# Amanda-Zheng/MR-GNAS

Hardware: AMD Instinct MI355X
Metric: million edges/sec per supernet fwd+bwd step (FB15k-237, dim=200) (higher is better)
Workload: dtype f32

## Files before the change

### mr-gnas_amd/csrc/mixedop.hip

```cpp
#include "common.hpp"

#define MRG_MIX_MAXK 8
static_assert(MRG_MIX_MAXK == MRG_MIX_MAX_CANDIDATES, "mrg_gated_branch.given is sized by the header's constant");

namespace mrg {

struct PtrPack { const float* p[MRG_MIX_MAXK]; };
struct MutPack { float* p[MRG_MIX_MAXK]; };
struct RowScalePack { const float* rs[MRG_MIX_MAXK]; float scale[MRG_MIX_MAXK]; float self_scale[MRG_MIX_MAXK]; int64_t edge_rows[MRG_MIX_MAXK]; int on[MRG_MIX_MAXK];
                      const float* full[MRG_MIX_MAXK];
                      const float* s[MRG_MIX_MAXK]; const float* gate[MRG_MIX_MAXK]; float* gs_out[MRG_MIX_MAXK]; int add_from[MRG_MIX_MAXK]; };

struct GatedPack { int k; const float* s; const float* c;
                   int pair_k;
                   int rk; const float* rf;
                   const float* rh; const float* uvc; int uld; int64_t b0, b1; float* rdq;
                   const int32_t* vrows;
                   int act; };

__device__ __forceinline__ int64_t valid_rows(const int32_t* vrows, int64_t rows) {
  if (vrows == nullptr) return rows;
  const int64_t v = (int64_t)*vrows;
  return v < rows ? (v < 0 ? 0 : v) : rows;
}
// ... 262 lines not shown
#pragma unroll
        for (int k = 0; k < KB; ++k) {
          vin[k] = Vec<VEC>::fill(0.f);
          if (k < K && ys.p[k]) vin[k] = Vec<VEC>::load(ys.p[k] + r * D + c * VEC);
        }
#pragma unroll
        for (int k = 0; k < KB; ++k) {
          if (k < K) {
            Vec<VEC> v = vin[k];
            if constexpr (GATED) {
              const bool isg = k == gp.k;
              const float cm = isg ? gck : (k == gp.rk ? rfv : 1.0f);
#pragma unroll
              for (int j = 0; j < VEC; ++j) v[j] = v[j] * (isg ? gsv[j] : 1.0f) * cm;
            }
            Vec<VEC> sc = Vec<VEC>::load(lds + (k * 2 + 0) * D + c * VEC), sh = Vec<VEC>::load(lds + (k * 2 + 1) * D + c * VEC);
            if constexpr (ACT == 0) {
#pragma unroll
              for (int j = 0; j < VEC; ++j) {
                float z = v[j] * sc[j] + sh[j];
                acc[j] += wk[k] * (z > 0.f ? z : 0.f);
              }
            } else {
#pragma unroll
              for (int j = 0; j < VEC; ++j) acc[j] += wk[k] * tanhf(v[j] * sc[j] + sh[j]);
            }
          }
        }
        if (pad) acc = Vec<VEC>::fill(0.f);
        acc.store(out + r * D + c * VEC);
      }
    }
  }
}

template <int VEC, int LPR, int KMAX, int KB, bool GATED, int ACT = 0>
__global__ __launch_bounds__(MRG_BLOCK) void mix_bwd_reduce_k(const float* __restrict__ g, PtrPack ys, int K,
                                                              const float* __restrict__ coef, const float* __restrict__ w,
                                                              float* __restrict__ ws, int64_t rows, int D, GatedPack gp) {
  rows = valid_rows(gp.vrows, rows);
  extern __shared__ float lds[];
  constexpr int RPB = MRG_BLOCK / LPR;
  constexpr int WIDTH = LPR * KMAX * VEC;
  const int sl = threadIdx.x % LPR, rw = row_group_of_thread<LPR>();
  const int dv = D / VEC;
  float* red = lds + K * 4 * D;
  for (int t = threadIdx.x; t < K * 4 * D; t += MRG_BLOCK) lds[t] = coef[t];
  __syncthreads();
  float wk[KB];
  Vec<VEC> a0[KB][KMAX], a1[KB][KMAX], a2[KB][KMAX];
#pragma unroll
  for (int k = 0; k < KB; ++k) {
    wk[k] = k < K ? w[k] : 0.f;
#pragma unroll
    for (int q = 0; q < KMAX; ++q) { a0[k][q] = Vec<VEC>::fill(0.f); a1[k][q] = Vec<VEC>::fill(0.f); a2[k][q] = Vec<VEC>::fill(0.f); }
  }
  for (int64_t r = (int64_t)blockIdx.x * RPB + rw; r < rows; r += (int64_t)gridDim.x * RPB) {
#pragma unroll
    for (int q = 0; q < KMAX; ++q) {
      int c = sl + q * LPR;
      if (c < dv) {
        float gck = 1.f, rfv = 1.f;
        Vec<VEC> gsv = Vec<VEC>::fill(0.f);
        if constexpr (GATED) {
          gck = gated_rowscale(gp, r);
          rfv = gp.rf[r];
          gsv = Vec<VEC>::load(gp.s + r * D + c * VEC);
        }
        Vec<VEC> gv = Vec<VEC>::load(g + r * D + c * VEC);
        Vec<VEC> vin[KB];
#pragma unroll
        for (int k = 0; k < KB; ++k) {
          vin[k] = Vec<VEC>::fill(0.f);
          if (k < K && ys.p[k]) vin[k] = Vec<VEC>::load(ys.p[k] + r * D + c * VEC);
        }
#pragma unroll
        for (int k = 0; k < KB; ++k) {
          if (k < K) {
            Vec<VEC> v = vin[k];
            if constexpr (GATED) {
              const bool isg = k == gp.k;
              const float cm = isg ? gck : (k == gp.rk ? rfv : 1.0f);
#pragma unroll
              for (int j = 0; j < VEC; ++j) v[j] = v[j] * (isg ? gsv[j] : 1.0f) * cm;
            }
            const float* cf = lds + k * 4 * D + c * VEC;
            const Vec<VEC> c0 = Vec<VEC>::load(cf), c1 = Vec<VEC>::load(cf + D), c2 = Vec<VEC>::load(cf + 2 * D), c3 = Vec<VEC>::load(cf + 3 * D);
#pragma unroll
            for (int j = 0; j < VEC; ++j) {
              float z = v[j] * c0[j] + c1[j];
              float xh = v[j] * c2[j] - c3[j];
              float rl, gr;
              if constexpr (ACT == 0) { rl = z > 0.f ? z : 0.f; gr = z > 0.f ? wk[k] * gv[j] : 0.f; }
              else { rl = tanhf(z); gr = wk[k] * gv[j] * (1.f - rl * rl); }
              a0[k][q][j] += gr;
              a1[k][q][j] += gr * xh;
              a2[k][q][j] += gv[j] * rl;
            }
          }
        }
      }
    }
  }
#pragma unroll
  for (int k = 0; k < KB; ++k) {
    if (k < K) {
      __syncthreads();
#pragma unroll
      for (int q = 0; q < KMAX; ++q) {
        int c = sl + q * LPR;
#pragma unroll
        for (int j = 0; j < VEC; ++j) {
          red[(rw * 3 + 0) * WIDTH + c * VEC + j] = a0[k][q][j];
          red[(rw * 3 + 1) * WIDTH + c * VEC + j] = a1[k][q][j];
          red[(rw * 3 + 2) * WIDTH + c * VEC + j] = a2[k][q][j];
        }
      }
      __syncthreads();
      float* dst = ws + ((int64_t)blockIdx.x * K + k) * 3 * D;
      for (int t = threadIdx.x; t < 3 * D; t += MRG_BLOCK) {
        int which = t / D, c = t - which * D;
        float acc = 0.f;
#pragma unroll
        for (int q2 = 0; q2 < RPB; ++q2) acc += red[(q2 * 3 + which) * WIDTH + c];
        dst[t] = acc;
      }
    }
  }
}

__global__ void mix_finalize_bwd_k(const float* __restrict__ red, int K, double total_rows, int D, float* __restrict__ coef2,
                                   MutPack dgamma, MutPack dbeta, float* __restrict__ dw, const int32_t* __restrict__ vrows) {
  if (vrows) total_rows = *vrows > 0 ? (double)*vrows : 1.0;
  __shared__ float part[256];
  int k = blockIdx.x;
  float accw = 0.f;
  for (int c = threadIdx.x; c < D; c += blockDim.x) {
    float s0 = red[(k * 3 + 0) * D + c], s1 = red[(k * 3 + 1) * D + c];
    coef2[(k * 2 + 0) * D + c] = (float)(s0 / total_rows);
    coef2[(k * 2 + 1) * D + c] = (float)(s1 / total_rows);
    if (dgamma.p[k]) dgamma.p[k][c] = s1;
    if (dbeta.p[k]) dbeta.p[k][c] = s0;
    accw += red[(k * 3 + 2) * D + c];
  }
  part[threadIdx.x] = accw;
  __syncthreads();
  if (threadIdx.x == 0) {
    float tot = 0.f;
    for (int i = 0; i < (int)blockDim.x; ++i) tot += part[i];
    dw[k] = tot;
  }
}

template <int VEC, int LPR, int KMAX, bool GATED, int KB, int ACT = 0>
__global__ __launch_bounds__(MRG_BLOCK) void mix_bwd_apply_k(const float* __restrict__ g, PtrPack ys, MutPack gys, int K,
                                                             const float* __restrict__ coef, const float* __restrict__ coef2,
                                                             const float* __restrict__ w, int64_t rows, int D, RowScalePack rsp,
                                                             GatedPack gp) {
  extern __shared__ float lds[];
  constexpr int RPB = MRG_BLOCK / LPR;
  const int sl = threadIdx.x % LPR, rw = row_group_of_thread<LPR>();
  const int dv = D / VEC;
  for (int t = threadIdx.x; t < K * 6 * D; t += MRG_BLOCK) {
    int k = t / (6 * D), rem = t - k * 6 * D;
    lds[t] = rem < 4 * D ? coef[(int64_t)k * 4 * D + rem] : coef2[(int64_t)k * 2 * D + rem - 4 * D];
  }
  __syncthreads();
  float wk[KB];
  bool need[KB];
#pragma unroll
  for (int k = 0; k < KB; ++k) {
    wk[k] = k < K ? w[k] : 0.f;
    need[k] = k < K && (gys.p[k] != nullptr || (GATED && k == gp.rk));
  }
#pragma unroll
  for (int k = 0; k < KB; ++k)
    if (k < K && rsp.on[k] == 2 && rsp.add_from[k] >= 0) {
#pragma unroll
      for (int q = 0; q < KB; ++q) if (q == rsp.add_from[k]) need[q] = true;
    }
  const bool hasr = GATED && gp.rk >= 0;
  const int64_t nvalid = valid_rows(gp.vrows, rows);
  for (int64_t r = (int64_t)blockIdx.x * RPB + rw; r < rows; r += (int64_t)gridDim.x * RPB) {
    const float live = r < nvalid ? 1.0f : 0.0f;
#pragma unroll
    for (int q = 0; q < KMAX; ++q) {
      const int c = sl + q * LPR;
      const bool act = c < dv;
      float gck = 1.f, rfv = 1.f, rhv = 0.f;
      Vec<VEC> gsv = Vec<VEC>::fill(0.f), gga = Vec<VEC>::fill(0.f), guv = Vec<VEC>::fill(0.f);
      Vec<VEC> ov[KB];
      Vec<VEC> orv = Vec<VEC>::fill(0.f);
      float dq = 0.f;
      float ckv[KB];
#pragma unroll
      for (int k = 0; k < KB; ++k) ckv[k] = 1.f;
      if (act) {
        if constexpr (GATED) {
          gck = gated_rowscale(gp, r);
          rfv = gp.rf[r];
          rhv = gp.rh[r];
          gsv = Vec<VEC>::load(gp.s + r * D + c * VEC);
          const int seg = (r >= gp.b0) + (r >= gp.b1);
          guv = Vec<VEC>::load(gp.uvc + (int64_t)seg * gp.uld + c * VEC);
        }
        Vec<VEC> gv = Vec<VEC>::load(g + r * D + c * VEC);
        Vec<VEC> vin[KB];
#pragma unroll
        for (int k = 0; k < KB; ++k) {
          vin[k] = Vec<VEC>::fill(0.f);
          if (k < K && need[k] && ys.p[k]) vin[k] = Vec<VEC>::load(ys.p[k] + r * D + c * VEC);
          if (k < K && rsp.on[k] && rsp.full[k]) ckv[k] = rsp.full[k][r];
        }
        if constexpr (GATED) {
#pragma unroll
          for (int k = 0; k < KB; ++k) {
            if (k == gp.k) {
              gga = vin[k];
#pragma unroll
              for (int j = 0; j < VEC; ++j) vin[k][j] = vin[k][j] * gsv[j] * gck;
            }
            if (k == gp.rk) {
#pragma unroll
              for (int j = 0; j < VEC; ++j) vin[k][j] = vin[k][j] * rfv;
            }
          }
        }
#pragma unroll
        for (int k = 0; k < KB; ++k) {
          ov[k] = Vec<VEC>::fill(0.f);
          if (k < K && need[k]) {
            const Vec<VEC> v = vin[k];
            const float* cf = lds + k * 6 * D + c * VEC;
            const Vec<VEC> c0 = Vec<VEC>::load(cf), c1 = Vec<VEC>::load(cf + D), c2 = Vec<VEC>::load(cf + 2 * D),
                           c3 = Vec<VEC>::load(cf + 3 * D), c4 = Vec<VEC>::load(cf + 4 * D), c5 = Vec<VEC>::load(cf + 5 * D);
#pragma unroll
            for (int j = 0; j < VEC; ++j) {
              float z = v[j] * c0[j] + c1[j];
              float xh = v[j] * c2[j] - c3[j];
              float gr;
              if constexpr (ACT == 0) gr = z > 0.f ? wk[k] * gv[j] : 0.f;
              else { const float th = tanhf(z); gr = wk[k] * gv[j] * (1.f - th * th); }
              ov[k][j] = (gr - c4[j] - xh * c5[j]) * c0[j] * live;
            }
          }
        }
        if (hasr) {
#pragma unroll
          for (int k = 0; k < KB; ++k) if (k == gp.rk) orv = ov[k];
#pragma unroll
          for (int j = 0; j < VEC; ++j) dq += orv[j] * gsv[j];
        }
      }
      float dzr = 0.f;
      if (hasr) {
        const float qr = group_sum<LPR>(dq);
        dzr = qr * rhv;
        if (sl == 0) gp.rdq[r] = qr;
      }
      if (act) {
#pragma unroll
        for (int k = 0; k < KB; ++k) {
          if (k < K && gys.p[k] != nullptr) {
            Vec<VEC> o = ov[k];
            if (rsp.on[k]) {
              const float ck = rsp.full[k] ? ckv[k]
                                           : (r < rsp.edge_rows[k] ? rsp.scale[k] * (rsp.rs[k] ? rsp.rs[k][r] : 1.0f) : rsp.self_scale[k]);
              if (rsp.on[k] == 2) {
                const Vec<VEC> sv = (GATED && k == gp.k) ? gsv : Vec<VEC>::load(rsp.s[k] + r * D + c * VEC);
                const Vec<VEC> ga = (GATED && k == gp.k) ? gga : Vec<VEC>::load(rsp.gate[k] + r * D + c * VEC);
                Vec<VEC> o2;
#pragma unroll
                for (int j = 0; j < VEC; ++j) {
                  const float gc = o[j] * ck;
                  o2[j] = gc * ga[j];
                  o[j] = gc * sv[j] * ga[j] * (1.0f - ga[j]);
                }
                const int af = rsp.add_from[k];
                if (af >= 0) {
#pragma unroll
                  for (int qq = 0; qq < KB; ++qq)
                    if (qq == af) {
#pragma unroll
                      for (int j = 0; j < VEC; ++j) o2[j] += ov[qq][j];
                    }
                }
                if (hasr && k == gp.k) {
#pragma unroll
                  for (int j = 0; j < VEC; ++j) o2[j] += orv[j] * rfv + dzr * guv[j];
                }
                o2.store(rsp.gs_out[k] + r * D + c * VEC);
              } else {
#pragma unroll
                for (int j = 0; j < VEC; ++j) o[j] = o[j] * ck;
              }
            }
            o.store(gys.p[k] + r * D + c * VEC);
          }
        }
      }
    }
  }
}


struct ZeroSrc { const float* ent; const float* rel; const int32_t* ei; const int32_t* ri; int op[4]; int K; const int32_t* vrows; };

template <int VEC>
__device__ __forceinline__ Vec<VEC> zero_val(int op, const Vec<VEC>& a, const Vec<VEC>& b) {
  Vec<VEC> y;
#pragma unroll
  for (int j = 0; j < VEC; ++j) y[j] = op == MRG_COMPOSE_MULT ? a[j] * b[j] : (op == MRG_COMPOSE_SUB ? a[j] - b[j] : a[j] + b[j]);
  return y;
}

constexpr int ZK = 3;

template <int VEC, int LPR, int KMAX>
__global__ __launch_bounds__(MRG_BLOCK) void zero_colstats_k(ZeroSrc z, int64_t rows, int D, double* __restrict__ ws) {
  rows = valid_rows(z.vrows, rows);
  constexpr int RPB = MRG_BLOCK / LPR;
  constexpr int WIDTH = LPR * KMAX * VEC;
  __shared__ double red[RPB * 2 * WIDTH];
  const int sl = threadIdx.x % LPR, rw = row_group_of_thread<LPR>();
  const int dv = D / VEC;
  const int K = z.K;
  double s1[ZK][KMAX][VEC], s2[ZK][KMAX][VEC];
#pragma unroll
  for (int k = 0; k < ZK; ++k)
#pragma unroll
    for (int q = 0; q < KMAX; ++q)
#pragma unroll
      for (int j = 0; j < VEC; ++j) { s1[k][q][j] = 0.0; s2[k][q][j] = 0.0; }
  const int64_t step = (int64_t)gridDim.x * RPB;
  int64_t r = (int64_t)blockIdx.x * RPB + rw;
  for (; r + 3 * step < rows; r += 4 * step) {
    const float* a[4]; const float* b[4];
#pragma unroll
    for (int u = 0; u < 4; ++u) { a[u] = z.ent + (int64_t)z.ei[r + u * step] * D; b[u] = z.rel + (int64_t)z.ri[r + u * step] * D; }
#pragma unroll
    for (int q = 0; q < KMAX; ++q) {
      int c = sl + q * LPR;
      if (c < dv) {
        Vec<VEC> va[4], vb[4];
#pragma unroll
        for (int u = 0; u < 4; ++u) { va[u] = Vec<VEC>::load(a[u] + c * VEC); vb[u] = Vec<VEC>::load(b[u] + c * VEC); }
#pragma unroll
        for (int u = 0; u < 4; ++u)
#pragma unroll
          for (int k = 0; k < ZK; ++k)
            if (k < K) {
              const Vec<VEC> y = zero_val<VEC>(z.op[k], va[u], vb[u]);
#pragma unroll
              for (int j = 0; j < VEC; ++j) { double d = (double)y[j]; s1[k][q][j] += d; s2[k][q][j] += d * d; }
            }
      }
    }
  }
  for (; r < rows; r += step) {
    const float* a = z.ent + (int64_t)z.ei[r] * D;
    const float* b = z.rel + (int64_t)z.ri[r] * D;
#pragma unroll
    for (int q = 0; q < KMAX; ++q) {
      int c = sl + q * LPR;
      if (c < dv) {
        const Vec<VEC> va = Vec<VEC>::load(a + c * VEC), vb = Vec<VEC>::load(b + c * VEC);
#pragma unroll
        for (int k = 0; k < ZK; ++k)
          if (k < K) {
            const Vec<VEC> y = zero_val<VEC>(z.op[k], va, vb);
#pragma unroll
            for (int j = 0; j < VEC; ++j) { double d = (double)y[j]; s1[k][q][j] += d; s2[k][q][j] += d * d; }
          }
      }
    }
  }
#pragma unroll
  for (int k = 0; k < ZK; ++k) {
    if (k < K) {
      __syncthreads();
#pragma unroll
      for (int q = 0; q < KMAX; ++q) {
        int c = sl + q * LPR;
#pragma unroll
        for (int j = 0; j < VEC; ++j) {
          red[(rw * 2 + 0) * WIDTH + c * VEC + j] = s1[k][q][j];
          red[(rw * 2 + 1) * WIDTH + c * VEC + j] = s2[k][q][j];
        }
      }
      __syncthreads();
      double* dst = ws + ((int64_t)blockIdx.x * K + k) * 2 * D;
      for (int t = threadIdx.x; t < 2 * D; t += MRG_BLOCK) {
        int which = t / D, c = t - which * D;
        double acc = 0.0;
#pragma unroll
        for (int q = 0; q < RPB; ++q) acc += red[(q * 2 + which) * WIDTH + c];
        dst[t] = acc;
      }
    }
  }
}

template <int VEC, int LPR, int KMAX>
__global__ __launch_bounds__(MRG_BLOCK) void zero_fwd_k(ZeroSrc z, const float* __restrict__ coef, const float* __restrict__ w,
                                                        float* __restrict__ out, int64_t rows, int D) {
  extern __shared__ float lds[];
  constexpr int RPB = MRG_BLOCK / LPR;
  const int sl = threadIdx.x % LPR, rw = row_group_of_thread<LPR>();
  const int dv = D / VEC;
  const int K = z.K;
  for (int t = threadIdx.x; t < K * 2 * D; t += MRG_BLOCK) {
    int k = t / (2 * D), rem = t - k * 2 * D;
    lds[t] = coef[(int64_t)k * 4 * D + rem];
  }
  __syncthreads();
  float wk[ZK];
#pragma unroll
  for (int k = 0; k < ZK; ++k) wk[k] = k < K ? w[k] : 0.f;
  const int64_t nvalid = valid_rows(z.vrows, rows);
  for (int64_t r = (int64_t)blockIdx.x * RPB + rw; r < rows; r += (int64_t)gridDim.x * RPB) {
    const float* a = z.ent + (int64_t)z.ei[r] * D;
    const float* b = z.rel + (int64_t)z.ri[r] * D;
    const bool pad = r >= nvalid;
#pragma unroll
    for (int q = 0; q < KMAX; ++q) {
      int c = sl + q * LPR;
      if (c < dv) {
        const Vec<VEC> va = Vec<VEC>::load(a + c * VEC), vb = Vec<VEC>::load(b + c * VEC);
        Vec<VEC> acc = Vec<VEC>::fill(0.f);
#pragma unroll
        for (int k = 0; k < ZK; ++k) {
          if (k < K) {
            const Vec<VEC> v = zero_val<VEC>(z.op[k], va, vb);
            Vec<VEC> sc = Vec<VEC>::load(lds + (k * 2 + 0) * D + c * VEC), sh = Vec<VEC>::load(lds + (k * 2 + 1) * D + c * VEC);
#pragma unroll
            for (int j = 0; j < VEC; ++j) {
              float zz = v[j] * sc[j] + sh[j];
              acc[j] += wk[k] * (zz > 0.f ? zz : 0.f);
            }
          }
        }
        if (pad) acc = Vec<VEC>::fill(0.f);
        acc.store(out + r * D + c * VEC);
      }
    }
  }
}

template <int VEC, int LPR, int KMAX>
__global__ __launch_bounds__(MRG_BLOCK) void zero_bwd_reduce_k(const float* __restrict__ g, ZeroSrc z, const float* __restrict__ coef,
                                                               const float* __restrict__ w, float* __restrict__ ws, int64_t rows, int D) {
// ... 301 lines not shown
  MutPack rm{}, rv{};
  for (int k = 0; k < K; ++k) {
    ga.p[k] = gamma_host[k]; be.p[k] = beta_host[k];
    rm.p[k] = rmean_host ? rmean_host[k] : nullptr;
    rv.p[k] = rvar_host ? rvar_host[k] : nullptr;
    if ((rm.p[k] == nullptr) != (rv.p[k] == nullptr)) return MRG_E_NULLPTR;
  }
  hipLaunchKernelGGL(mix_finalize_fwd_k, dim3((D + 127) / 128, K), dim3(128), 0, (hipStream_t)stream, sums, ga, be, rm, rv, K,
                     total_rows > 0 ? total_rows : 1.0, D, eps, momentum, coef, (const int32_t*)nullptr);
  MRG_LAUNCH_CHECK();
  return MRG_OK;
}

extern "C" int mrg_mix_fwd(const float* const* y_host, int K, const float* coef, const float* w, const float* addend, float* out,
                           int64_t rows, int D, const mrg_gated_branch* gated, void* stream) {
  if (!pack_ok((const void* const*)y_host, K) || rows < 0 || D <= 0) return MRG_E_SHAPE;
  if (rows == 0) return MRG_OK;
  if (!coef || !w || !out) return MRG_E_NULLPTR;
  hipStream_t st = (hipStream_t)stream;
  PtrPack ys{};
  bool al = aligned16(out) && aligned16(addend);
  for (int k = 0; k < K; ++k) { ys.p[k] = y_host[k]; al = al && aligned16(y_host[k]); }
  GatedPack gp;
  const int grc = gated_pack(gated, y_host, K, &gp, &al);
  if (grc != MRG_OK) return grc;
  RowGeom g = row_geom(D, al);
  if (!g.ok) return MRG_E_SHAPE;
  size_t lds = (size_t)K * 2 * D * sizeof(float);
  if (lds > 64 * 1024) return MRG_E_SHAPE;
#define CALL(V, L, KM)                                                                                    \
  do {                                                                                                    \
    const dim3 grid_(mix_fwd_grid(rows, L));                                                               \
    if (gp.act == 1) {                                                                                    \
      hipLaunchKernelGGL((mix_fwd_k<V, L, KM, false, 5, 1>), grid_, dim3(MRG_BLOCK), lds, st, ys, K, coef, w, out, rows, D, addend, gp); \
    } else if (gp.k >= 0 || gp.rk >= 0) {                                                                        \
      if (K <= 5) hipLaunchKernelGGL((mix_fwd_k<V, L, KM, true, 5>), grid_, dim3(MRG_BLOCK), lds, st, ys, K, coef, w, out, rows, D, addend, gp); \
      else hipLaunchKernelGGL((mix_fwd_k<V, L, KM, true, MRG_MIX_MAXK>), grid_, dim3(MRG_BLOCK), lds, st, ys, K, coef, w, out, rows, D, addend, gp); \
    } else {                                                                                              \
      if (K <= 5) hipLaunchKernelGGL((mix_fwd_k<V, L, KM, false, 5>), grid_, dim3(MRG_BLOCK), lds, st, ys, K, coef, w, out, rows, D, addend, gp); \
      else hipLaunchKernelGGL((mix_fwd_k<V, L, KM, false, MRG_MIX_MAXK>), grid_, dim3(MRG_BLOCK), lds, st, ys, K, coef, w, out, rows, D, addend, gp); \
    }                                                                                                     \
  } while (0)
  MRG_DISPATCH_GEOM(g, CALL);
#undef CALL
  MRG_LAUNCH_CHECK();
  return MRG_OK;
}

extern "C" int mrg_mix_bwd_reduce(const float* g, const float* const* y_host, int K, const float* coef, const float* w, float* red,
                                  void* ws, int64_t rows, int D, const mrg_gated_branch* gated, void* stream) {
  if (!pack_ok((const void* const*)y_host, K) || rows < 0 || D <= 0) return MRG_E_SHAPE;
  if (!coef || !w || !red || (rows > 0 && !g)) return MRG_E_NULLPTR;
  if (!ws) return MRG_E_WORKSPACE;
  hipStream_t st = (hipStream_t)stream;
  PtrPack ys{};
  bool al = aligned16(g);
  for (int k = 0; k < K; ++k) { ys.p[k] = y_host[k]; al = al && aligned16(y_host[k]); }
  GatedPack gp;
  const int grc = gated_pack(gated, y_host, K, &gp, &al);
  if (grc != MRG_OK) return grc;
  RowGeom gm = row_geom(D, al);
  if (!gm.ok) return MRG_E_SHAPE;
  int grid = 1;
#define CALL(V, L, KM)                                                                                    \
  do {                                                                                                    \
    grid = mix_reduce_grid(rows, L);                                                                             \
    size_t lds = ((size_t)K * 4 * D + (size_t)(MRG_BLOCK / L) * 3 * (L * KM * V)) * sizeof(float);        \
    if (lds > 64 * 1024) return MRG_E_SHAPE;                                                              \
    if (gp.act == 1) hipLaunchKernelGGL((mix_bwd_reduce_k<V, L, KM, 5, false, 1>), dim3(grid), dim3(MRG_BLOCK), lds, st, g, ys, K, coef, w, (float*)ws, rows, D, gp); \
    else if ((gp.k >= 0 || gp.rk >= 0) && K <= 5) hipLaunchKernelGGL((mix_bwd_reduce_k<V, L, KM, 5, true>), dim3(grid), dim3(MRG_BLOCK), lds, st, g, ys, K, coef, w, (float*)ws, rows, D, gp); \
    else if (gp.k >= 0 || gp.rk >= 0) hipLaunchKernelGGL((mix_bwd_reduce_k<V, L, KM, MRG_MIX_MAXK, true>), dim3(grid), dim3(MRG_BLOCK), lds, st, g, ys, K, coef, w, (float*)ws, rows, D, gp); \
    else if (K <= 4) hipLaunchKernelGGL((mix_bwd_reduce_k<V, L, KM, 4, false>), dim3(grid), dim3(MRG_BLOCK), lds, st, g, ys, K, coef, w, (float*)ws, rows, D, gp); \
    else hipLaunchKernelGGL((mix_bwd_reduce_k<V, L, KM, MRG_MIX_MAXK, false>), dim3(grid), dim3(MRG_BLOCK), lds, st, g, ys, K, coef, w, (float*)ws, rows, D, gp); \
  } while (0)
  MRG_DISPATCH_GEOM(gm, CALL);
#undef CALL
  MRG_LAUNCH_CHECK();
  int len = K * 3 * D;
  launch_ordered_reduce<float>((const float*)ws, red, 0, grid, len, len, st);
  MRG_LAUNCH_CHECK();
  return MRG_OK;
}

extern "C" int mrg_mix_finalize_bwd(const float* red, int K, double total_rows, int D, float* coef2, float* const* dgamma_host,
                                    float* const* dbeta_host, float* dw, const int32_t* valid_rows, void* stream) {
  if (K < 1 || K > MRG_MIX_MAXK || D <= 0) return MRG_E_SHAPE;
  if (valid_rows && !(total_rows >= 0 && total_rows == (double)(int64_t)total_rows)) return MRG_E_SHAPE;
  if (!red || !coef2 || !dw) return MRG_E_NULLPTR;
  MutPack dg{}, db{};
  for (int k = 0; k < K; ++k) {
    dg.p[k] = dgamma_host ? dgamma_host[k] : nullptr;
    db.p[k] = dbeta_host ? dbeta_host[k] : nullptr;
  }
  hipLaunchKernelGGL(mix_finalize_bwd_k, dim3(K), dim3(256), 0, (hipStream_t)stream, red, K, total_rows > 0 ? total_rows : 1.0, D,
                     coef2, dg, db, dw, valid_rows);
  MRG_LAUNCH_CHECK();
  return MRG_OK;
}

extern "C" int mrg_mix_bwd_apply(const float* g, const float* const* y_host, float* const* gy_host, int K, const float* coef,
                                 const float* coef2, const float* w, const float* const* rs_host, const float* rs_scale_host,
                                 const float* rs_self_host, const int64_t* rs_edge_rows_host, const int* rs_on_host,
                                 const float* const* rs_full_host,
                                 const float* const* fold_s_host, const float* const* fold_gate_host, float* const* fold_gs_host,
                                 const int* fold_add_from_host, int64_t rows, int D, const mrg_gated_branch* gated, void* stream) {
  if (!pack_ok((const void* const*)y_host, K) || !gy_host || rows < 0 || D <= 0) return MRG_E_SHAPE;
  if (rows == 0) return MRG_OK;
  if (!g || !coef || !coef2 || !w) return MRG_E_NULLPTR;
  hipStream_t st = (hipStream_t)stream;
  PtrPack ys{};
  MutPack gys{};
  bool al = aligned16(g);
  bool any = false;
  for (int k = 0; k < K; ++k) {
    ys.p[k] = y_host[k]; gys.p[k] = gy_host[k];
    al = al && aligned16(y_host[k]) && aligned16(gy_host[k]);
    any = any || gy_host[k] != nullptr;
  }
  if (!any) return MRG_OK;
  RowScalePack rsp{};
  for (int k = 0; k < MRG_MIX_MAXK; ++k) rsp.add_from[k] = -1;
  if (rs_on_host) {
    if (!rs_scale_host || !rs_self_host || !rs_edge_rows_host) return MRG_E_NULLPTR;
    for (int k = 0; k < K; ++k) {
      rsp.on[k] = rs_on_host[k];
      rsp.rs[k] = rs_host ? rs_host[k] : nullptr;
      rsp.full[k] = (rs_full_host && rsp.on[k]) ? rs_full_host[k] : nullptr;
      rsp.scale[k] = rs_scale_host[k]; rsp.self_scale[k] = rs_self_host[k]; rsp.edge_rows[k] = rs_edge_rows_host[k];
      if (rsp.on[k] == 2) {
        if (!fold_s_host || !fold_gate_host || !fold_gs_host || !fold_s_host[k] || !fold_gate_host[k] || !fold_gs_host[k]) return MRG_E_NULLPTR;
        rsp.s[k] = fold_s_host[k]; rsp.gate[k] = fold_gate_host[k]; rsp.gs_out[k] = fold_gs_host[k];
        if (fold_add_from_host && fold_add_from_host[k] >= 0) {
          const int q = fold_add_from_host[k];
          if (q >= K || q == k || !y_host[q] || y_host[q] != rsp.s[k]) return MRG_E_SHAPE;
          rsp.add_from[k] = q;
          any = true;
        }
        al = al && aligned16(rsp.s[k]) && aligned16(rsp.gate[k]) && aligned16(rsp.gs_out[k]);
      } else if (rsp.on[k] != 0 && rsp.on[k] != 1) {
        return MRG_E_ENUM;
      }
    }
  }
  GatedPack gp;
  const int grc = gated_pack(gated, y_host, K, &gp, &al, true);
  if (grc != MRG_OK) return grc;
  if (gp.k >= 0 && rsp.on[gp.k] == 2 && (rsp.s[gp.k] != gp.s || rsp.gate[gp.k] != y_host[gp.k])) return MRG_E_SHAPE;
  if (gp.rk >= 0 && (gp.k < 0 || rsp.on[gp.k] != 2 || gy_host[gp.rk] != nullptr)) return MRG_E_SHAPE;
  RowGeom gm = row_geom(D, al);
  if (!gm.ok) return MRG_E_SHAPE;
  if (gp.rk >= 0 && gm.kmax != 1) return MRG_E_SHAPE;
  size_t lds = (size_t)K * 6 * D * sizeof(float);
  if (lds > 64 * 1024) return MRG_E_SHAPE;
#define CALL(V, L, KM)                                                                                    \
  do {                                                                                                    \
    const dim3 grid_(mix_apply_grid(rows, L));                                                             \
    if (gp.act == 1) {                                                                                    \
      hipLaunchKernelGGL((mix_bwd_apply_k<V, L, KM, false, 5, 1>), grid_, dim3(MRG_BLOCK), lds, st, g, ys, gys, K, coef, coef2, w, rows, D, rsp, gp); \
    } else if (gp.k >= 0 || gp.rk >= 0) {                                                                        \
      if (K <= 5) hipLaunchKernelGGL((mix_bwd_apply_k<V, L, KM, true, 5>), grid_, dim3(MRG_BLOCK), lds, st, g, ys, gys, K, coef, coef2, w, rows, D, rsp, gp); \
      else hipLaunchKernelGGL((mix_bwd_apply_k<V, L, KM, true, MRG_MIX_MAXK>), grid_, dim3(MRG_BLOCK), lds, st, g, ys, gys, K, coef, coef2, w, rows, D, rsp, gp); \
    } else {                                                                                              \
      if (K <= 5) hipLaunchKernelGGL((mix_bwd_apply_k<V, L, KM, false, 5>), grid_, dim3(MRG_BLOCK), lds, st, g, ys, gys, K, coef, coef2, w, rows, D, rsp, gp); \
      else hipLaunchKernelGGL((mix_bwd_apply_k<V, L, KM, false, MRG_MIX_MAXK>), grid_, dim3(MRG_BLOCK), lds, st, g, ys, gys, K, coef, coef2, w, rows, D, rsp, gp); \
    }                                                                                                     \
  } while (0)
  MRG_DISPATCH_GEOM(gm, CALL);
#undef CALL
  MRG_LAUNCH_CHECK();
  return MRG_OK;
}


static int zero_src(ZeroSrc* z, const float* ent, const float* rel, const int32_t* ei, const int32_t* ri, const int* ops_host, int K) {
  if (K < 1 || K > ZK || !ops_host) return MRG_E_SHAPE;
  if (!ent || !rel || !ei || !ri) return MRG_E_NULLPTR;
  z->ent = ent; z->rel = rel; z->ei = ei; z->ri = ri; z->K = K;
  for (int k = 0; k < K; ++k) {
    if (ops_host[k] < 0 || ops_host[k] > 2) return MRG_E_ENUM;
    z->op[k] = ops_host[k];
  }
  return MRG_OK;
}

static int zero_grid(int64_t rows, int lpr) {
  int64_t b = row_blocks(rows, lpr, 8);
  return (int)(b > 2048 ? 2048 : b);
}

extern "C" int64_t mrg_zero_workspace_bytes(int D) {
  if (D <= 0) return 0;
  return (int64_t)2048 * ZK * 3 * D * sizeof(double);
}

static int zero_colstats_blocks(const ZeroSrc& z, int64_t rows, int D, void* ws, hipStream_t st, int* grid_out) {
  if (rows < 0 || D <= 0) return MRG_E_SHAPE;
  if (!ws) return MRG_E_WORKSPACE;
  RowGeom g = row_geom(D, aligned16(z.ent) && aligned16(z.rel));
  if (!g.ok) return MRG_E_SHAPE;
  int grid = 1;
#define CALL(V, L, KM)                                                                                    \
  do {                                                                                                    \
    grid = zero_grid(rows, L);                                                                             \
    hipLaunchKernelGGL((zero_colstats_k<V, L, KM>), dim3(grid), dim3(MRG_BLOCK), 0, st, z, rows, D, (double*)ws); \
  } while (0)
  MRG_DISPATCH_GEOM(g, CALL);
#undef CALL
  MRG_LAUNCH_CHECK();
  *grid_out = grid;
  return MRG_OK;
}

extern "C" int mrg_zero_colstats(const float* ent, const float* rel, const int32_t* ent_idx, const int32_t* rel_idx, const int* ops_host, int K,
                                 int64_t rows, int D, double* sums, void* ws, void* stream) {
  ZeroSrc z{};
  int rc = zero_src(&z, ent, rel, ent_idx, rel_idx, ops_host, K);
  if (rc != MRG_OK) return rc;
  if (!sums) return MRG_E_NULLPTR;
  hipStream_t st = (hipStream_t)stream;
  int grid = 1;
  rc = zero_colstats_blocks(z, rows, D, ws, st, &grid);
  if (rc != MRG_OK) return rc;
  const int len = K * 2 * D;
  launch_ordered_reduce<double>((const double*)ws, sums, 0, grid, len, len, st);
  MRG_LAUNCH_CHECK();
  return MRG_OK;
}

extern "C" int mrg_zero_stats_coef(const float* ent, const float* rel, const int32_t* ent_idx, const int32_t* rel_idx, const int* ops_host, int K,
                                   const float* const* gamma_host, const float* const* beta_host, float* const* rmean_host,
                                   float* const* rvar_host, int64_t rows, double total_rows, int D, float eps, float momentum, float* coef,
                                   void* ws, const int32_t* valid_rows, void* stream) {
  ZeroSrc z{};
  z.vrows = valid_rows;
  int rc = zero_src(&z, ent, rel, ent_idx, rel_idx, ops_host, K);
  if (rc != MRG_OK) return rc;
  if (D <= 0 || total_rows < 0) return MRG_E_SHAPE;
  if (valid_rows && total_rows != (double)rows) return MRG_E_SHAPE;
  if (!coef || !gamma_host || !beta_host) return MRG_E_NULLPTR;
  hipStream_t st = (hipStream_t)stream;
  int grid = 1;
  rc = zero_colstats_blocks(z, rows, D, ws, st, &grid);
  if (rc != MRG_OK) return rc;
  PtrPack ga{}, be{};
  MutPack rm{}, rv{};
  for (int k = 0; k < K; ++k) {
    ga.p[k] = gamma_host[k]; be.p[k] = beta_host[k];
    rm.p[k] = rmean_host ? rmean_host[k] : nullptr;
    rv.p[k] = rvar_host ? rvar_host[k] : nullptr;
    if ((rm.p[k] == nullptr) != (rv.p[k] == nullptr)) return MRG_E_NULLPTR;
  }
  hipLaunchKernelGGL(mix_reduce_finalize_fwd_k, dim3((D + 63) / 64, K), dim3(1024), 0, st, (const double*)ws, grid, ga, be, rm, rv, K,
                     total_rows > 0 ? total_rows : 1.0, D, eps, momentum, coef, valid_rows);
  MRG_LAUNCH_CHECK();
  return MRG_OK;
}

extern "C" int mrg_zero_fwd(const float* ent, const float* rel, const int32_t* ent_idx, const int32_t* rel_idx, const int* ops_host, int K,
                            const float* coef, const float* w, float* out, int64_t rows, int D, const int32_t* valid_rows,
                            void* stream) {
  ZeroSrc z{};
  z.vrows = valid_rows;
  const int rc = zero_src(&z, ent, rel, ent_idx, rel_idx, ops_host, K);
  if (rc != MRG_OK) return rc;
  if (rows < 0 || D <= 0) return MRG_E_SHAPE;
  if (rows == 0) return MRG_OK;
  if (!coef || !w || !out) return MRG_E_NULLPTR;
  hipStream_t st = (hipStream_t)stream;
  RowGeom g = row_geom(D, aligned16(ent) && aligned16(rel) && aligned16(out));
  if (!g.ok) return MRG_E_SHAPE;
  const size_t lds = (size_t)K * 2 * D * sizeof(float);
  if (lds > 64 * 1024) return MRG_E_SHAPE;
#define CALL(V, L, KM)                                                                                    \
  hipLaunchKernelGGL((zero_fwd_k<V, L, KM>), dim3(grid_for(rows, (MRG_BLOCK / L) * 4)), dim3(MRG_BLOCK), lds, st, z, coef, w, out, rows, D)
  MRG_DISPATCH_GEOM(g, CALL);
#undef CALL
  MRG_LAUNCH_CHECK();
  return MRG_OK;
}

extern "C" int mrg_zero_bwd_reduce(const float* g, const float* ent, const float* rel, const int32_t* ent_idx, const int32_t* rel_idx,
                                   const int* ops_host, int K, const float* coef, const float* w, float* red, void* ws, int64_t rows, int D,
                                   const int32_t* valid_rows, void* stream) {
  ZeroSrc z{};
  z.vrows = valid_rows;
  const int rc = zero_src(&z, ent, rel, ent_idx, rel_idx, ops_host, K);
  if (rc != MRG_OK) return rc;
  if (rows < 0 || D <= 0) return MRG_E_SHAPE;
  if (!coef || !w || !red || (rows > 0 && !g)) return MRG_E_NULLPTR;
  if (!ws) return MRG_E_WORKSPACE;
  hipStream_t st = (hipStream_t)stream;
  RowGeom gm = row_geom(D, aligned16(g) && aligned16(ent) && aligned16(rel));
  if (!gm.ok) return MRG_E_SHAPE;
  int grid = 1;
#define CALL(V, L, KM)                                                                                    \
  do {                                                                                                    \
    grid = zero_grid(rows, L);                                                                             \
    size_t lds = ((size_t)K * 4 * D + (size_t)(MRG_BLOCK / L) * 3 * (L * KM * V)) * sizeof(float);        \
    if (lds > 64 * 1024) return MRG_E_SHAPE;                                                              \
    hipLaunchKernelGGL((zero_bwd_reduce_k<V, L, KM>), dim3(grid), dim3(MRG_BLOCK), lds, st, g, z, coef, w, (float*)ws, rows, D); \
  } while (0)
  MRG_DISPATCH_GEOM(gm, CALL);
#undef CALL
  MRG_LAUNCH_CHECK();
  const int len = K * 3 * D;
  launch_ordered_reduce<float>((const float*)ws, red, 0, grid, len, len, st);
  MRG_LAUNCH_CHECK();
  return MRG_OK;
}

extern "C" int mrg_zero_bwd_apply(const float* g, const float* ent, const float* rel, const int32_t* ent_idx, const int32_t* rel_idx,
                                  const int* ops_host, int K, const float* coef, const float* coef2, const float* w, float* g_ent_rows,
                                  float* g_rel_rows, int64_t rows, int D, const int32_t* valid_rows, void* stream) {
  ZeroSrc z{};
  z.vrows = valid_rows;
  const int rc = zero_src(&z, ent, rel, ent_idx, rel_idx, ops_host, K);
  if (rc != MRG_OK) return rc;
  if (rows < 0 || D <= 0) return MRG_E_SHAPE;
  if (rows == 0 || (!g_ent_rows && !g_rel_rows)) return MRG_OK;
  if (!g || !coef || !coef2 || !w) return MRG_E_NULLPTR;
  hipStream_t st = (hipStream_t)stream;
// ... 12 lines not shown
```

Measured before the change: 11.57.

## Specialize mixed-op backward apply kernel by resolved candidate roles

The generic backward apply kernel looped over all K candidates, using per-candidate runtime branches and register arrays sized for the maximum candidate count. The host now classifies candidates into gated, row, added and plain roles and launches a kernel templated on that layout, so only the needed loads and math are compiled and register pressure drops. A generic fallback kernel with unroll 1 and on-the-fly recomputation handles unresolved layouts. Explicit fma and contract-off helpers try to reproduce the old rounding, which adds code size and some risk of small numerical mismatches.

```diff
diff --git a/mr-gnas_amd/csrc/mixedop.hip b/mr-gnas_amd/csrc/mixedop.hip
--- a/mr-gnas_amd/csrc/mixedop.hip
+++ b/mr-gnas_amd/csrc/mixedop.hip
@@ -438,11 +438,102 @@
   }
 }
 
-template <int VEC, int LPR, int KMAX, bool GATED, int KB, int ACT = 0>
-__global__ __launch_bounds__(MRG_BLOCK) void mix_bwd_apply_k(const float* __restrict__ g, PtrPack ys, MutPack gys, int K,
-                                                             const float* __restrict__ coef, const float* __restrict__ coef2,
-                                                             const float* __restrict__ w, int64_t rows, int D, RowScalePack rsp,
-                                                             GatedPack gp) {
+template <int VEC, int ACT>
+__device__ __forceinline__ Vec<VEC> apply_gy(const Vec<VEC>& v, const Vec<VEC>& gv, const float* cf, int D, float wk, float live, bool first) {
+#pragma clang fp contract(off)
+  const Vec<VEC> c0 = Vec<VEC>::load(cf), c1 = Vec<VEC>::load(cf + D), c2 = Vec<VEC>::load(cf + 2 * D),
+                 c3 = Vec<VEC>::load(cf + 3 * D), c4 = Vec<VEC>::load(cf + 4 * D), c5 = Vec<VEC>::load(cf + 5 * D);
+  Vec<VEC> o;
+#pragma unroll
+  for (int j = 0; j < VEC; ++j) {
+    const float z = __builtin_fmaf(v[j], c0[j], c1[j]);
+    float xh = __builtin_fmaf(v[j], c2[j], -c3[j]);
+    if (VEC == 1 && ACT == 0) xh = v[j] * c2[j] - c3[j];
+    else if (ACT == 0 && (j & 1)) xh = first ? v[j] * c2[j] - c3[j] : xh;
+    float t;
+    if constexpr (ACT == 0) {
+      const float gr = z > 0.f ? wk * gv[j] : 0.f;
+      t = __builtin_fmaf(-xh, c5[j], gr - c4[j]);
+    } else {
+      const float th = tanhf(z);
+      const float wg = wk * gv[j], om = __builtin_fmaf(-th, th, 1.f);
+      t = __builtin_fmaf(-xh, c5[j], __builtin_fmaf(wg, om, -c4[j]));
+      if (VEC == 4 && j == 3) t = first ? (wg * om - c4[j]) - xh * c5[j] : t;
+    }
+    o[j] = t * c0[j] * live;
+  }
+  return o;
+}
+
+template <int VEC>
+__device__ __forceinline__ void apply_gated(const Vec<VEC>& gy, float ck, const Vec<VEC>& sv, const Vec<VEC>& ga, Vec<VEC>& dzv, Vec<VEC>& o2) {
+#pragma clang fp contract(off)
+#pragma unroll
+  for (int j = 0; j < VEC; ++j) {
+    const float gc = gy[j] * ck;
+    o2[j] = gc * ga[j];
+    dzv[j] = gc * sv[j] * ga[j] * (1.0f - ga[j]);
+  }
+}
+
+template <int VEC>
+__device__ __forceinline__ void apply_row_term(Vec<VEC>& o2, const Vec<VEC>& orv, float rfv, float dzr, const Vec<VEC>& guv) {
+#pragma clang fp contract(off)
+#pragma unroll
+  for (int j = 0; j < VEC; ++j) o2[j] = o2[j] + __builtin_fmaf(orv[j], rfv, dzr * guv[j]);
+}
+
+template <int VEC>
+__device__ __forceinline__ float apply_row_dot(const Vec<VEC>& orv, const Vec<VEC>& sv) {
+#pragma clang fp contract(off)
+  float dq = 0.f;
+#pragma unroll
+  for (int j = 0; j < VEC; ++j) dq = dq + orv[j] * sv[j];
+  return dq;
+}
+
+template <int VEC>
+__device__ __forceinline__ Vec<VEC> apply_scaled(const Vec<VEC>& a, float x) {
+#pragma clang fp contract(off)
+  Vec<VEC> o;
+#pragma unroll
+  for (int j = 0; j < VEC; ++j) o[j] = a[j] * x;
+  return o;
+}
+
+template <int VEC>
+__device__ __forceinline__ Vec<VEC> apply_sum(const Vec<VEC>& a, const Vec<VEC>& b) {
+#pragma clang fp contract(off)
+  Vec<VEC> o;
+#pragma unroll
+  for (int j = 0; j < VEC; ++j) o[j] = a[j] + b[j];
+  return o;
+}
+
+template <int VEC>
+__device__ __forceinline__ Vec<VEC> apply_gate_value(const Vec<VEC>& ga, const Vec<VEC>& sv, float gck) {
+#pragma clang fp contract(off)
+  Vec<VEC> o;
+#pragma unroll
+  for (int j = 0; j < VEC; ++j) o[j] = ga[j] * sv[j] * gck;
+  return o;
+}
+
+constexpr int APPLY_NO = 5;
+struct ApplySlots { int g, r, a, o[APPLY_NO]; };
+struct ApplyOther { const float* y; float* gy; const float* full; };
+template <int NO> struct ApplyOthers { ApplyOther o[NO]; };
+
+template <int VEC, int LPR, int KMAX, int ACT, bool HG, bool HR, bool HA, int NO>
+__global__ __launch_bounds__(MRG_BLOCK) void mix_bwd_apply_k(
+    const float* __restrict__ g, const float* __restrict__ coef, const float* __restrict__ coef2, const float* __restrict__ w, int K,
+    int64_t rows, int D, const int32_t* __restrict__ vrows, ApplySlots slot, int n_oth, ApplyOthers<NO> oth,
+    const float* __restrict__ gate, const float* __restrict__ s, const float* __restrict__ c, const float* __restrict__ ck,
+    float* __restrict__ dz, float* __restrict__ gs_out,
+    const float* __restrict__ rf, const float* __restrict__ rh, const float* __restrict__ uvc, int uld, int64_t b0, int64_t b1,
+    float* __restrict__ rdq) {
+  static_assert(!HR || (HG && KMAX == 1), "the row dot is one group_sum over the row's lanes; its gradient goes into gs_out");
+  static_assert(!HA || HG, "the added candidate goes into the gated candidate's gs_out");
   extern __shared__ float lds[];
   constexpr int RPB = MRG_BLOCK / LPR;
   const int sl = threadIdx.x % LPR, rw = row_group_of_thread<LPR>();
@@ -452,90 +543,142 @@
     lds[t] = rem < 4 * D ? coef[(int64_t)k * 4 * D + rem] : coef2[(int64_t)k * 2 * D + rem - 4 * D];
   }
   __syncthreads();
-  float wk[KB];
-  bool need[KB];
-#pragma unroll
-  for (int k = 0; k < KB; ++k) {
-    wk[k] = k < K ? w[k] : 0.f;
-    need[k] = k < K && (gys.p[k] != nullptr || (GATED && k == gp.rk));
-  }
-#pragma unroll
-  for (int k = 0; k < KB; ++k)
-    if (k < K && rsp.on[k] == 2 && rsp.add_from[k] >= 0) {
-#pragma unroll
-      for (int q = 0; q < KB; ++q) if (q == rsp.add_from[k]) need[q] = true;
-    }
-  const bool hasr = GATED && gp.rk >= 0;
+  const int n = HG ? NO : n_oth;
+  const bool first0 = slot.o[0] == 0;
+  float wg = 0.f, wr = 0.f, wa = 0.f, wo[NO];
+  const float* cfo[NO];
+  if constexpr (HG) wg = w[slot.g];
+  if constexpr (HR) wr = w[slot.r];
+  if constexpr (HA) wa = w[slot.a];
+#pragma unroll
+  for (int i = 0; i < NO; ++i) {
+    wo[i] = i < n ? w[slot.o[i]] : 0.f;
+    cfo[i] = lds + (i < n ? slot.o[i] : 0) * 6 * D;
+  }
+  const float* cfg = lds + (HG ? slot.g : 0) * 6 * D;
+  const float* cfr = lds + (HR ? slot.r : 0) * 6 * D;
+  const float* cfa = lds + (HA ? slot.a : 0) * 6 * D;
+  const int64_t nvalid = valid_rows(vrows, rows);
+  const int64_t step = (int64_t)gridDim.x * RPB;
+  for (int64_t r = (int64_t)blockIdx.x * RPB + rw; r < rows; r += step) {
+    const float live = r < nvalid ? 1.0f : 0.0f;
+    const int64_t ro = r * D;
+    float gck = 1.f, ckv = 1.f, rfv = 1.f, rhv = 0.f, fo[NO];
+    const float* urow = uvc;
+    if constexpr (HG) { gck = c[r]; ckv = ck[r]; }
+    if constexpr (HR) {
+      rfv = rf[r];
+      rhv = rh[r];
+      urow = uvc + (int64_t)((r >= b0) + (r >= b1)) * uld;
+    }
+#pragma unroll
+    for (int i = 0; i < NO; ++i) fo[i] = (HG && i < n && oth.o[i].full) ? oth.o[i].full[r] : 1.f;
+#pragma unroll
+    for (int q = 0; q < KMAX; ++q) {
+      const int cc = sl + q * LPR;
+      const bool act = cc < dv;
+      const int off = cc * VEC;
+      Vec<VEC> gsv, gga, guv, ovg, ova, orv, ovo[NO];
+      float dq = 0.f;
+      if (act) {
+        if constexpr (HG) { gsv = Vec<VEC>::load(s + ro + off); gga = Vec<VEC>::load(gate + ro + off); }
+        if constexpr (HR) guv = Vec<VEC>::load(urow + off);
+        const Vec<VEC> gv = Vec<VEC>::load(g + ro + off);
+        Vec<VEC> vo[NO];
+#pragma unroll
+        for (int i = 0; i < NO; ++i) {
+          vo[i] = Vec<VEC>::fill(0.f);
+          if (i < n && oth.o[i].y) vo[i] = Vec<VEC>::load(oth.o[i].y + ro + off);
+        }
+        if constexpr (HG) ovg = apply_gy<VEC, ACT>(apply_gate_value<VEC>(gga, gsv, gck), gv, cfg + off, D, wg, live, false);
+        if constexpr (HA) ova = apply_gy<VEC, ACT>(gsv, gv, cfa + off, D, wa, live, false);
+        if constexpr (HR) {
+          orv = apply_gy<VEC, ACT>(apply_scaled<VEC>(gsv, rfv), gv, cfr + off, D, wr, live, false);
+          dq = apply_row_dot<VEC>(orv, gsv);
+        }
+#pragma unroll
+        for (int i = 0; i < NO; ++i)
+          if (i < n) ovo[i] = apply_gy<VEC, ACT>(vo[i], gv, cfo[i] + off, D, wo[i], live, !HG && i == 0 && first0);
+      }
+      float dzr = 0.f;
+      if constexpr (HR) {
+        const float qr = group_sum<LPR>(dq);
+        dzr = qr * rhv;
+        if (sl == 0) rdq[r] = qr;
+      }
+      if (act) {
+#pragma unroll
+        for (int i = 0; i < NO; ++i)
+          if (i < n) {
+            Vec<VEC> o = ovo[i];
+            if (HG && oth.o[i].full) o = apply_scaled<VEC>(o, fo[i]);
+            o.store(oth.o[i].gy + ro + off);
+          }
+        if constexpr (HG) {
+          Vec<VEC> dzv, o2;
+          apply_gated<VEC>(ovg, ckv, gsv, gga, dzv, o2);
+          if constexpr (HA) o2 = apply_sum<VEC>(o2, ova);
+          if constexpr (HR) apply_row_term<VEC>(o2, orv, rfv, dzr, guv);
+          o2.store(gs_out + ro + off);
+          dzv.store(dz + ro + off);
+        }
+      }
+    }
+  }
+}
+
+template <int VEC>
+struct ApplyAny {
+  const PtrPack& ys; const RowScalePack& rsp; const GatedPack& gp;
+  const float* lds; const float* w; int D; int act;
+  __device__ __forceinline__ Vec<VEC> gy(int k, int64_t r, int64_t ro, int off, const Vec<VEC>& gv, const Vec<VEC>& gsv, float live, Vec<VEC>* raw) const {
+    Vec<VEC> v = Vec<VEC>::fill(0.f);
+    const float* y = ys.p[k];
+    if (y) v = Vec<VEC>::load(y + ro + off);
+    *raw = v;
+    if (k == gp.k) v = apply_gate_value<VEC>(v, gsv, gp.c[r]);
+    if (k == gp.rk) v = apply_scaled<VEC>(v, gp.rf[r]);
+    const float* cf = lds + k * 6 * D + off;
+    return act == 1 ? apply_gy<VEC, 1>(v, gv, cf, D, w[k], live, k == 0) : apply_gy<VEC, 0>(v, gv, cf, D, w[k], live, k == 0);
+  }
+};
+
+template <int VEC, int LPR, int KMAX>
+__global__ __launch_bounds__(MRG_BLOCK) void mix_bwd_apply_any_k(const float* __restrict__ g, PtrPack ys, MutPack gys, int K,
+                                                                 const float* __restrict__ coef, const float* __restrict__ coef2,
+                                                                 const float* __restrict__ w, int64_t rows, int D, RowScalePack rsp,
+                                                                 GatedPack gp) {
+  extern __shared__ float lds[];
+  constexpr int RPB = MRG_BLOCK / LPR;
+  const int sl = threadIdx.x % LPR, rw = row_group_of_thread<LPR>();
+  const int dv = D / VEC;
+  for (int t = threadIdx.x; t < K * 6 * D; t += MRG_BLOCK) {
+    int k = t / (6 * D), rem = t - k * 6 * D;
+    lds[t] = rem < 4 * D ? coef[(int64_t)k * 4 * D + rem] : coef2[(int64_t)k * 2 * D + rem - 4 * D];
+  }
+  __syncthreads();
+  const ApplyAny<VEC> any{ys, rsp, gp, lds, w, D, gp.act};
+  const bool hass = gp.k >= 0 || gp.rk >= 0, hasr = KMAX == 1 && gp.rk >= 0;
   const int64_t nvalid = valid_rows(gp.vrows, rows);
   for (int64_t r = (int64_t)blockIdx.x * RPB + rw; r < rows; r += (int64_t)gridDim.x * RPB) {
     const float live = r < nvalid ? 1.0f : 0.0f;
-#pragma unroll
+    const int64_t ro = r * D;
+#pragma unroll 1
     for (int q = 0; q < KMAX; ++q) {
-      const int c = sl + q * LPR;
-      const bool act = c < dv;
-      float gck = 1.f, rfv = 1.f, rhv = 0.f;
-      Vec<VEC> gsv = Vec<VEC>::fill(0.f), gga = Vec<VEC>::fill(0.f), guv = Vec<VEC>::fill(0.f);
-      Vec<VEC> ov[KB];
-      Vec<VEC> orv = Vec<VEC>::fill(0.f);
-      float dq = 0.f;
-      float ckv[KB];
-#pragma unroll
-      for (int k = 0; k < KB; ++k) ckv[k] = 1.f;
+      const int cc = sl + q * LPR;
+      const bool act = cc < dv;
+      const int off = cc * VEC;
+      Vec<VEC> gsv = Vec<VEC>::fill(0.f), guv, gv, orv, raw;
+      float rfv = 1.f, rhv = 0.f, dq = 0.f;
       if (act) {
-        if constexpr (GATED) {
-          gck = gated_rowscale(gp, r);
+        gv = Vec<VEC>::load(g + ro + off);
+        if (hass) gsv = Vec<VEC>::load(gp.s + ro + off);
+        if (hasr) {
           rfv = gp.rf[r];
           rhv = gp.rh[r];
-          gsv = Vec<VEC>::load(gp.s + r * D + c * VEC);
-          const int seg = (r >= gp.b0) + (r >= gp.b1);
-          guv = Vec<VEC>::load(gp.uvc + (int64_t)seg * gp.uld + c * VEC);
-        }
-        Vec<VEC> gv = Vec<VEC>::load(g + r * D + c * VEC);
-        Vec<VEC> vin[KB];
-#pragma unroll
-        for (int k = 0; k < KB; ++k) {
-          vin[k] = Vec<VEC>::fill(0.f);
-          if (k < K && need[k] && ys.p[k]) vin[k] = Vec<VEC>::load(ys.p[k] + r * D + c * VEC);
-          if (k < K && rsp.on[k] && rsp.full[k]) ckv[k] = rsp.full[k][r];
-        }
-        if constexpr (GATED) {
-#pragma unroll
-          for (int k = 0; k < KB; ++k) {
-            if (k == gp.k) {
-              gga = vin[k];
-#pragma unroll
-              for (int j = 0; j < VEC; ++j) vin[k][j] = vin[k][j] * gsv[j] * gck;
-            }
-            if (k == gp.rk) {
-#pragma unroll
-              for (int j = 0; j < VEC; ++j) vin[k][j] = vin[k][j] * rfv;
-            }
-          }
-        }
-#pragma unroll
-        for (int k = 0; k < KB; ++k) {
-          ov[k] = Vec<VEC>::fill(0.f);
-          if (k < K && need[k]) {
-            const Vec<VEC> v = vin[k];
-            const float* cf = lds + k * 6 * D + c * VEC;
-            const Vec<VEC> c0 = Vec<VEC>::load(cf), c1 = Vec<VEC>::load(cf + D), c2 = Vec<VEC>::load(cf + 2 * D),
-                           c3 = Vec<VEC>::load(cf + 3 * D), c4 = Vec<VEC>::load(cf + 4 * D), c5 = Vec<VEC>::load(cf + 5 * D);
-#pragma unroll
-            for (int j = 0; j < VEC; ++j) {
-              float z = v[j] * c0[j] + c1[j];
-              float xh = v[j] * c2[j] - c3[j];
-              float gr;
-              if constexpr (ACT == 0) gr = z > 0.f ? wk[k] * gv[j] : 0.f;
-              else { const float th = tanhf(z); gr = wk[k] * gv[j] * (1.f - th * th); }
-              ov[k][j] = (gr - c4[j] - xh * c5[j]) * c0[j] * live;
-            }
-          }
-        }
-        if (hasr) {
-#pragma unroll
-          for (int k = 0; k < KB; ++k) if (k == gp.rk) orv = ov[k];
-#pragma unroll
-          for (int j = 0; j < VEC; ++j) dq += orv[j] * gsv[j];
+          guv = Vec<VEC>::load(gp.uvc + (int64_t)((r >= gp.b0) + (r >= gp.b1)) * gp.uld + off);
+          orv = any.gy(gp.rk, r, ro, off, gv, gsv, live, &raw);
+          dq = apply_row_dot<VEC>(orv, gsv);
         }
       }
       float dzr = 0.f;
@@ -545,44 +688,33 @@
         if (sl == 0) gp.rdq[r] = qr;
       }
       if (act) {
-#pragma unroll
-        for (int k = 0; k < KB; ++k) {
-          if (k < K && gys.p[k] != nullptr) {
-            Vec<VEC> o = ov[k];
-            if (rsp.on[k]) {
-              const float ck = rsp.full[k] ? ckv[k]
-                                           : (r < rsp.edge_rows[k] ? rsp.scale[k] * (rsp.rs[k] ? rsp.rs[k][r] : 1.0f) : rsp.self_scale[k]);
-              if (rsp.on[k] == 2) {
-                const Vec<VEC> sv = (GATED && k == gp.k) ? gsv : Vec<VEC>::load(rsp.s[k] + r * D + c * VEC);
-                const Vec<VEC> ga = (GATED && k == gp.k) ? gga : Vec<VEC>::load(rsp.gate[k] + r * D + c * VEC);
-                Vec<VEC> o2;
-#pragma unroll
-                for (int j = 0; j < VEC; ++j) {
-                  const float gc = o[j] * ck;
-                  o2[j] = gc * ga[j];
-                  o[j] = gc * sv[j] * ga[j] * (1.0f - ga[j]);
-                }
-                const int af = rsp.add_from[k];
-                if (af >= 0) {
-#pragma unroll
-                  for (int qq = 0; qq < KB; ++qq)
-                    if (qq == af) {
-#pragma unroll
-                      for (int j = 0; j < VEC; ++j) o2[j] += ov[qq][j];
-                    }
-                }
-                if (hasr && k == gp.k) {
-#pragma unroll
-                  for (int j = 0; j < VEC; ++j) o2[j] += orv[j] * rfv + dzr * guv[j];
-                }
-                o2.store(rsp.gs_out[k] + r * D + c * VEC);
-              } else {
-#pragma unroll
-                for (int j = 0; j < VEC; ++j) o[j] = o[j] * ck;
-              }
+#pragma unroll 1
+        for (int k = 0; k < K; ++k) {
+          float* dst = gys.p[k];
+          if (dst == nullptr) continue;
+          Vec<VEC> o = any.gy(k, r, ro, off, gv, gsv, live, &raw);
+          const int on = rsp.on[k];
+          if (on) {
+            const float* full = rsp.full[k];
+            float ckv;
+            if (full) ckv = full[r];
+            else if (r < rsp.edge_rows[k]) { const float* rs = rsp.rs[k]; ckv = rsp.scale[k] * (rs ? rs[r] : 1.0f); }
+            else ckv = rsp.self_scale[k];
+            if (on == 2) {
+              const Vec<VEC> sv = k == gp.k ? gsv : Vec<VEC>::load(rsp.s[k] + ro + off);
+              const Vec<VEC> ga = k == gp.k ? raw : Vec<VEC>::load(rsp.gate[k] + ro + off);
+              Vec<VEC> dzv, o2;
+              apply_gated<VEC>(o, ckv, sv, ga, dzv, o2);
+              const int af = rsp.add_from[k];
+              if (af >= 0) o2 = apply_sum<VEC>(o2, any.gy(af, r, ro, off, gv, gsv, live, &raw));
+              if (hasr && k == gp.k) apply_row_term<VEC>(o2, orv, rfv, dzr, guv);
+              o2.store(rsp.gs_out[k] + ro + off);
+              o = dzv;
+            } else {
+              o = apply_scaled<VEC>(o, ckv);
             }
-            o.store(gys.p[k] + r * D + c * VEC);
           }
+          o.store(dst + ro + off);
         }
       }
     }
@@ -1190,21 +1322,47 @@
   if (gp.rk >= 0 && gm.kmax != 1) return MRG_E_SHAPE;
   size_t lds = (size_t)K * 6 * D * sizeof(float);
   if (lds > 64 * 1024) return MRG_E_SHAPE;
+  ApplySlots slot{-1, -1, -1, {0, 0, 0, 0, 0}};
+  ApplyOthers<APPLY_NO> oth{};
+  int n_oth = 0;
+  const int G = gp.k, R = gp.rk, A = G >= 0 ? rsp.add_from[G] : -1;
+  bool resolved = K <= 5;
+  if (G >= 0) resolved = resolved && rsp.on[G] == 2 && rsp.full[G] && gy_host[G];
+  if (A >= 0) resolved = resolved && gy_host[A] == nullptr;
+  for (int k = 0; k < K && resolved; ++k) {
+    if (k == G || k == R || k == A) continue;
+    if (rsp.on[k] == 2 || (rsp.on[k] == 1 && (!rsp.full[k] || G < 0))) resolved = false;
+    else if (gy_host[k]) {
+      slot.o[n_oth] = k;
+      oth.o[n_oth++] = ApplyOther{y_host[k], gy_host[k], rsp.on[k] ? rsp.full[k] : nullptr};
+    }
+  }
+  slot.g = G; slot.r = R; slot.a = A;
+  if (G >= 0 && (G == 0 || R == 0 || A == 0 || (n_oth > 0 && slot.o[0] == 0))) resolved = false;
+  const int layout = !resolved ? -1 : G < 0 ? 0 : (R >= 0 && A >= 0 && n_oth == 1) ? 1 : (R < 0 && A >= 0 && n_oth == 2) ? 2
+                                                  : (R >= 0 && A < 0 && n_oth == 2) ? 3 : -1;
+#define ROLE(V, L, KM, ACT, HG, HR, HA, NO)                                                                                        \
+  do {                                                                                                                             \
+    ApplyOthers<NO> o_{};                                                                                                          \
+    for (int i = 0; i < NO; ++i) o_.o[i] = oth.o[i];                                                                                \
+    hipLaunchKernelGGL((mix_bwd_apply_k<V, L, KM, ACT, HG, HR, HA, NO>), grid_, dim3(MRG_BLOCK), lds, st, g, coef, coef2, w, K, rows, D, \
+                       gp.vrows, slot, n_oth, o_, G >= 0 ? y_host[G] : nullptr, gp.s, gp.c, G >= 0 ? rsp.full[G] : nullptr,          \
+                       G >= 0 ? gy_host[G] : nullptr, G >= 0 ? rsp.gs_out[G] : nullptr, gp.rf, gp.rh, gp.uvc, gp.uld, gp.b0, gp.b1,    \
+                       gp.rdq);                                                                                                    \
+  } while (0)
 #define CALL(V, L, KM)                                                                                    \
   do {                                                                                                    \
     const dim3 grid_(mix_apply_grid(rows, L));                                                             \
-    if (gp.act == 1) {                                                                                    \
-      hipLaunchKernelGGL((mix_bwd_apply_k<V, L, KM, false, 5, 1>), grid_, dim3(MRG_BLOCK), lds, st, g, ys, gys, K, coef, coef2, w, rows, D, rsp, gp); \
-    } else if (gp.k >= 0 || gp.rk >= 0) {                                                                        \
-      if (K <= 5) hipLaunchKernelGGL((mix_bwd_apply_k<V, L, KM, true, 5>), grid_, dim3(MRG_BLOCK), lds, st, g, ys, gys, K, coef, coef2, w, rows, D, rsp, gp); \
-      else hipLaunchKernelGGL((mix_bwd_apply_k<V, L, KM, true, MRG_MIX_MAXK>), grid_, dim3(MRG_BLOCK), lds, st, g, ys, gys, K, coef, coef2, w, rows, D, rsp, gp); \
-    } else {                                                                                              \
-      if (K <= 5) hipLaunchKernelGGL((mix_bwd_apply_k<V, L, KM, false, 5>), grid_, dim3(MRG_BLOCK), lds, st, g, ys, gys, K, coef, coef2, w, rows, D, rsp, gp); \
-      else hipLaunchKernelGGL((mix_bwd_apply_k<V, L, KM, false, MRG_MIX_MAXK>), grid_, dim3(MRG_BLOCK), lds, st, g, ys, gys, K, coef, coef2, w, rows, D, rsp, gp); \
-    }                                                                                                     \
+    if (layout == 0 && gp.act == 1) ROLE(V, L, KM, 1, false, false, false, APPLY_NO);                      \
+    else if (layout == 0) ROLE(V, L, KM, 0, false, false, false, APPLY_NO);                                \
+    else if (layout == 2) ROLE(V, L, KM, 0, true, false, true, 2);                                         \
+    else if (layout == 1) ROLE(V, L, 1, 0, true, true, true, 1);           \
+    else if (layout == 3) ROLE(V, L, 1, 0, true, true, false, 2);                                          \
+    else hipLaunchKernelGGL((mix_bwd_apply_any_k<V, L, KM>), grid_, dim3(MRG_BLOCK), lds, st, g, ys, gys, K, coef, coef2, w, rows, D, rsp, gp); \
   } while (0)
   MRG_DISPATCH_GEOM(gm, CALL);
 #undef CALL
+#undef ROLE
   MRG_LAUNCH_CHECK();
   return MRG_OK;
 }
```

After: 11.70, median of 6. 1.1% higher.
